# Neptune-Crypto/twenty-first

Hardware: AMD Instinct MI355X
Metric: goldilocks_ntt_gfelts_per_s (higher is better)
Workload: dtype u64

## Files before the change

### include/tf_hip.h

```cpp
#ifndef TF_HIP_H
#define TF_HIP_H

#include <stddef.h>
#include <stdint.h>

#ifdef __cplusplus
extern "C" {
#endif

enum tf_status {
    TF_OK = 0,
    TF_ERR_TOO_FEW_LEAFS = 1,
    TF_ERR_INCORRECT_NUMBER_OF_LEAFS = 2,
    TF_ERR_TREE_TOO_HIGH = 3,
    TF_ERR_LEN_NOT_POWER_OF_TWO = 4,
    TF_ERR_LEN_TOO_LARGE = 5,
    TF_ERR_ORDER_NOT_ABOVE_DEGREE = 6,
    TF_ERR_NULL_POINTER = 7,
    TF_ERR_NO_DEVICE = 8,
    TF_ERR_HIP = 9,
    TF_ERR_OUT_OF_MEMORY = 10,
    TF_ERR_LEAF_INDEX_INVALID = 11,
    TF_ERR_INVERSE_OF_ZERO = 12,
    TF_ERR_BUFFER_TOO_SMALL = 13,
// ... 333 lines not shown
    TF_FIELD_OP_ADD_SUB2 = 4,
    TF_FIELD_OP_ADD_SUB_LAZY2 = 5,
    TF_FIELD_OP_ADD_LAZY4 = 6,
    TF_FIELD_OP_SUB_LAZY4 = 7,
    TF_FIELD_OP_MONT_MUL2 = 8,
    TF_FIELD_OP_MONT_MUL3 = 9,
    TF_FIELD_OP_MONT_MUL4 = 10,
    TF_FIELD_OP_CANONICAL = 11,
    TF_FIELD_OP_MX_FOLD4_CANON = 12,
    TF_FIELD_OP_MX_FOLD4_LAZY = 13,
    TF_FIELD_OP_MX_FOLD2 = 14,
    TF_FIELD_OP_COUNT = 15
};
int tf_debug_field_op_dev(int op, const uint64_t *d_a, const uint64_t *d_b, uint64_t *d_out0, uint64_t *d_out1, size_t count, void *stream);

enum { TF_NTT_NETWORK_FORM_COUNT = 42 };
int tf_debug_ntt_network_dev(int form, uint64_t *d_x, size_t count, void *stream);
void tf_debug_ntt_network_config(int *lazy, int *asm_bfly, int *asm_pow2, int *pow2_wide);

#ifdef __cplusplus
}
#endif
#endif
```

### twenty-first_amd/csrc/ntt_kernels.h

```cpp
#pragma once

#include <type_traits>

#include "gl64.h"
#include "ntt_args.h"
#include "ntt_network.h"

namespace tfk {

using gl::u32;
using gl::u64;

struct NttPassArgs {
    const u64* in;
    u64* out;
    const u64* inner_tw;
    const u64* post_tw;
    const u64* pre_scale;
    long long n_out;
    const u64* in2;
    const u64* post_scale;
    long long js_i0, js_i1, js_i2, js_c, js_k;
    long long n_coeffs;
    long long ps_i1;
    long long ib0, ib1, ib2, ob0, ob1, ob2;
    long long in_cs_hi, out_cs_hi;
    long long in_rs, out_rs;
    long long tw_rs;
    long long ps_rs;
    u32 d1, d2;
    u32 d01;
// ... 47 lines not shown
    return ((u64)v[1] << 32) | v[0];
}
__device__ __forceinline__ u64 buf_load_tab(__amdgpu_buffer_rsrc_t r, u32 voff, u32 soff) {
    const tf_v2u v = __builtin_amdgcn_raw_buffer_load_b64(r, voff, soff, 0);
    return ((u64)v[1] << 32) | v[0];
}
template <int AUX = TF_STORE_AUX>
__device__ __forceinline__ void buf_store(__amdgpu_buffer_rsrc_t r, u32 voff, u32 soff, u64 x) {
    tf_v2u v;
    v[0] = (u32)x;
    v[1] = (u32)(x >> 32);
    __builtin_amdgcn_raw_buffer_store_b64(v, r, voff, soff, AUX);
}


template <bool INV, int Q0, bool TRUNC = false, bool SCALED = false>
__device__ __forceinline__ void tail_p5(u64 (&x)[32], bool act, char* obase, u32 toff, long long out_rs_bytes, int qlim = 32,
                                        const char* sbase = nullptr, u32 soff = 0, long long s_rs_bytes = 0, bool nt = false) {
    DitRange<INV, 5, Q0, Q0 + 4, false>::run(x);
    if (act) {
        const __amdgpu_buffer_rsrc_t ro = buf_rsrc(obase);
        if constexpr (SCALED) {
            u64 w[8];
#pragma unroll
            for (int i = 0; i < 4; ++i) {
                w[i] = *reinterpret_cast<const u64*>(sbase + (long long)(32 * (Q0 + i)) * s_rs_bytes + soff);
                w[4 + i] = *reinterpret_cast<const u64*>(sbase + (long long)(32 * (Q0 + i + 16)) * s_rs_bytes + soff);
            }
#pragma unroll
            for (int i = 0; i < 4; ++i) gl::mont_mul2(x[Q0 + i], w[i], x[Q0 + i + 16], w[4 + i], x[Q0 + i], x[Q0 + i + 16]);
        }
        (void)nt;
#pragma unroll
// ... 195 lines not shown
        }
    }
    const bool act_in = LAST1024 ? (c_in < ncv) : act;
    int ch_in = ch, cl_in = cl;
    if constexpr (LAST1024) {
        const int w = col0 + c_in + (col0 + c_in < 0 ? A.col_wrap : 0);
        const int e = (int)div_by_L((u32)w, L);
        ch_in = e - ch0, cl_in = w - e * L;
    }

    unsigned long long stamp[6];
    if constexpr (MODE == 3) stamp[0] = __builtin_readcyclecounter();
    u64 x[32];
#pragma unroll
    for (int q = 0; q < 32; ++q) x[q] = 0;
    constexpr bool LDS_TW = TF_LDS_TW && MODE == 0;
    u64* const ltw = lds + (LAST1024 ? kL1024ExchangeWords : 32 * s1_);
    if constexpr (LDS_TW) {
        if ((LAST1024 || R1024) || A.inner_tw) {
            const u64* itw = A.inner_tw + ((PRE2 || PRE4) ? (int)half * 1024 : 0);
            for (int i = t; i < 32 * P2; i += blockDim.x) ltw[(i >> 5) * kLdsTwStride + (i & 31)] = itw[i];
            __syncthreads();
        }
    }
    __builtin_amdgcn_s_setprio(TF_PRIO_LOAD);
    if constexpr (MODE == 1) {
#pragma unroll
        for (int q = 0; q < 32; ++q) x[q] = (u64)(t * 32 + q) * 0x9e3779b97f4a7c15ULL >> 1;
#ifdef TF_AB_BUILD
    } else if (PRE4 && act_in) {
// ... 131 lines not shown
        } else {
#pragma unroll
        for (int q = 0; q < 32; ++q) x[q] = ld(slot_off(q));
#pragma unroll
        for (int q0 = 0; q0 < 32; q0 += 8) {
            u64 w[8];
#pragma unroll
            for (int i = 0; i < 8; ++i) w[i] = ld(slot_off(q0 + i) + poff);
            scale8(w);
            if (q0 == 0) pre2_combine8<INV, 0>(x, w, half != 0);
            else if (q0 == 8) pre2_combine8<INV, 8>(x, w, half != 0);
            else if (q0 == 16) pre2_combine8<INV, 16>(x, w, half != 0);
            else pre2_combine8<INV, 24>(x, w, half != 0);
        }
        }
    } else if (act_in) {
        const u32 toff = (u32)(((long long)ch_in * A.in_cs_hi + cl_in + (long long)g_in * A.in_rs) * 8);
        const char* base = reinterpret_cast<const char*>(in);
        if constexpr ((LAST1024 || COLP) && SCALE != 1) {
            const __amdgpu_buffer_rsrc_t ri = buf_rsrc(in);
#pragma unroll
            for (int q = 0; q < 32; ++q) x[q] = buf_load<LAST1024 ? TF_AUX_LAST_LOAD : TF_LOAD_AUX>(ri, toff, (u32)((long long)(brev5(q) << p2) * A.in_rs * 8));
        } else
#pragma unroll
        for (int q = 0; q < 32; ++q) {
            const long long ur = (long long)(brev5(q) << p2);
            const u64* ptr = reinterpret_cast<const u64*>(base + ur * A.in_rs * 8 + toff);
            if constexpr (SCALE == 1) {
                const long long j = (ur + g) * A.ps_rs + (A.ps_col ? bcol : 0);
                if (A.n_coeffs < 0 || j < A.n_coeffs) x[q] = *ptr;
// ... 44 lines not shown
    __builtin_amdgcn_s_setprio(0);
    if constexpr (MODE != 2 && !(PRE2 && TF_PRE2_BURST16 == 2 && SCALE != 1)) {
        dit_half<INV, 0, LAZY1>(x);
        __builtin_amdgcn_sched_barrier(0);
    }
    if constexpr (MODE == 3) {
        stamp[1] = __builtin_readcyclecounter();
        asm volatile("s_waitcnt vmcnt(0)" ::: "memory");
        stamp[2] = __builtin_readcyclecounter();
    }
    if constexpr (MODE != 2) {
        dit_half<INV, 16, LAZY1>(x);
        dit_level<INV, 5, LAZY1>(x);
        if ((LAST1024 || R1024) || A.inner_tw) {
            const u64* tw = LDS_TW ? ltw + g_in * kLdsTwStride : A.inner_tw + g_in * 32;
#pragma unroll
            for (int q = 0; q < 32; q += 4) mul4_inplace(x, q, tw[q], tw[q + 1], tw[q + 2], tw[q + 3]);
        }
    }
    if constexpr (MODE == 3) { asm volatile("" :: "v"(x[0]), "v"(x[31])); stamp[3] = __builtin_readcyclecounter(); }
    if constexpr (LAST1024) {
        constexpr int S1 = kL1024S1, CS = kL1024CS;
        const int wround = c_in >> 3, wcc = c_in & 7, rround = c >> 3, rcc = c & 7;
        u64* wr = lds + wcc * CS + g_in;
        const u64* rd = lds + g * S1 + rcc * CS;
        const int nr = (A.nc + 7) >> 3;
#pragma unroll 1
        for (int r = 0; r < nr; ++r) {
            if (r) __syncthreads();
            if (wround == r) {
#pragma unroll
                for (int q = 0; q < 32; ++q) wr[q * S1] = x[q];
// ... 20 lines not shown
            if (myround == r) {
#pragma unroll
                for (int q = 0; q < 32; ++q) {
                    const int s = q >> p2;
                    const int gbr = q & (P2 - 1);
                    const int gg = p2 ? (int)(__brev((unsigned)gbr) >> (32 - p2)) : 0;
                    const int k1 = g + (s << p2);
                    x[q] = rd[k1 * s1_ + gg * s2_];
                }
            }
        }
    }
    if constexpr (MODE == 3) { asm volatile("" :: "v"(x[0]), "v"(x[31])); stamp[4] = __builtin_readcyclecounter(); }
    __builtin_amdgcn_s_setprio(TF_PRIO_STEP2);
    if constexpr (LAST1024) {
        dit_half<INV, 0>(x);
        dit_half<INV, 16>(x);
        const u32 toff = (u32)(((long long)ch * A.out_cs_hi + cl + (long long)g * A.out_rs) * 8);
        char* base = reinterpret_cast<char*>(out);
        if constexpr (SCALE == 2) {
            long long j0 = (long long)i0 * A.js_i0 + (long long)i1 * A.js_i1 + (long long)(ch0 + ch) * A.js_c + (long long)g * A.js_k;
            if constexpr (PRE2) j0 += (long long)half * A.pre2_js_off;
            const char* sb = reinterpret_cast<const char*>(A.post_scale);
            const u32 soff = (u32)(j0 * 8);
            tail_p5<INV, 0, false, true>(x, act, base, toff, A.out_rs * 8, 32, sb, soff, A.js_k * 8);
            tail_p5<INV, 4, false, true>(x, act, base, toff, A.out_rs * 8, 32, sb, soff, A.js_k * 8);
            tail_p5<INV, 8, false, true>(x, act, base, toff, A.out_rs * 8, 32, sb, soff, A.js_k * 8);
            tail_p5<INV, 12, false, true>(x, act, base, toff, A.out_rs * 8, 32, sb, soff, A.js_k * 8);
            return;
        }
        if (A.n_out >= 0) {
            const long long j0 = (long long)i0 * A.js_i0 + (long long)i1 * A.js_i1 + (long long)(ch0 + ch) * A.js_c + (long long)g * A.js_k;
            const long long rem = A.n_out - j0, step = 32 * A.js_k;
            const int qlim = rem <= 0 ? 0 : (int)min(32ll, (rem + step - 1) / step);
            tail_p5<INV, 0, true>(x, act, base, toff, A.out_rs * 8, qlim);
            tail_p5<INV, 4, true>(x, act, base, toff, A.out_rs * 8, qlim);
            tail_p5<INV, 8, true>(x, act, base, toff, A.out_rs * 8, qlim);
            tail_p5<INV, 12, true>(x, act, base, toff, A.out_rs * 8, qlim);
            return;
        }
        const bool nts = (A.nt & 2) != 0;
        tail_p5<INV, 0>(x, act, base, toff, A.out_rs * 8, 32, nullptr, 0, 0, nts);
        tail_p5<INV, 4>(x, act, base, toff, A.out_rs * 8, 32, nullptr, 0, 0, nts);
        tail_p5<INV, 8>(x, act, base, toff, A.out_rs * 8, 32, nullptr, 0, 0, nts);
        tail_p5<INV, 12>(x, act, base, toff, A.out_rs * 8, 32, nullptr, 0, 0, nts);
        return;
    }
    if constexpr (MODE != 2) {
        if (p2 >= 1) dit_level<INV, 1, LAZY2>(x);
        if (p2 >= 2) dit_level<INV, 2, LAZY2>(x);
        if (p2 >= 3) dit_level<INV, 3, LAZY2>(x);
        if (p2 >= 4) dit_level<INV, 4, LAZY2>(x);
        if (p2 >= 5) dit_level<INV, 5, LAZY2>(x);
    }
    if constexpr (MODE == 1) {
        u64 acc = 0;
#pragma unroll
        for (int q = 0; q < 32; ++q) acc ^= x[q];
        if (acc == 0x123456789abcdefULL) out[t] = acc;
    } else if (act) {
// ... 939 lines not shown
```

### twenty-first_amd/csrc/ntt_network.h

```cpp
#pragma once

#include "gl64.h"

namespace tfk {

using gl::u32;
using gl::u64;

template <bool INV, int LVL, int J>
struct TwExp {
    static constexpr int fwd = ((39 << (6 - LVL)) * J) % 192;
    static constexpr int value = INV ? (192 - fwd) % 192 : fwd;
};

#ifndef TF_ASM_BFLY
#define TF_ASM_BFLY 1
#endif
#ifndef TF_LDS_TW
#define TF_LDS_TW 1
#endif
constexpr int kLdsTwStride = 34;
constexpr int kR1024Nc = 16, kR1024Cpr = 8, kR1024Rounds = 2, kR1024S1 = 264;
constexpr int kL1024S1 = 273, kL1024CS = 34;
constexpr int kL1024ExchangeWords = ((31 * kL1024S1 + 7 * kL1024CS + 32 + 1) / 2) * 2;
#ifndef TF_LAZY
#define TF_LAZY 1
#endif

template <bool INV, int LVL, int I>
struct Bf {
    static constexpr int H = 1 << (LVL - 1);
    static constexpr int j = I % H;
    static constexpr int ia = (I / H) * 2 * H + j;
    static constexpr int ib = ia + H;
    static constexpr int E = TwExp<INV, LVL, j>::value;
    static constexpr bool neg = gl::Pow2Mul<E>::negate;
};

template <int E, bool LAZY_IN>
__device__ __forceinline__ u64 tw_operand(u64 b) {
    if constexpr (E % 192 == 0) {
// ... 143 lines not shown
        if constexpr (I + 2 < END) DitRange<INV, LVL, I + 2, END, LAZY>::run(x);
#endif
    }
};
template <bool INV, int LVL, bool LAZY = false, int WIDE = TF_POW2_WIDE>
__device__ __forceinline__ void dit_level(u64 (&x)[32]) { DitRange<INV, LVL, 0, 16, LAZY && TF_LAZY, WIDE>::run(x); }

template <bool INV, int FIRST, bool LAZY = false, int WIDE = TF_POW2_WIDE>
__device__ __forceinline__ void dit_half(u64 (&x)[32]) {
    DitRange<INV, 1, FIRST / 2, FIRST / 2 + 8, LAZY && TF_LAZY, WIDE>::run(x);
    DitRange<INV, 2, FIRST / 2, FIRST / 2 + 8, LAZY && TF_LAZY, WIDE>::run(x);
    DitRange<INV, 3, FIRST / 2, FIRST / 2 + 8, LAZY && TF_LAZY, WIDE>::run(x);
    DitRange<INV, 4, FIRST / 2, FIRST / 2 + 8, LAZY && TF_LAZY, WIDE>::run(x);
}

__device__ __forceinline__ void mul4_inplace(u64 (&x)[32], int q0, u64 w0, u64 w1, u64 w2, u64 w3) {
    const u64 a4[4] = {x[q0], x[q0 + 1], x[q0 + 2], x[q0 + 3]}, b4[4] = {w0, w1, w2, w3};
    u64 r4[4];
    gl::mont_mul4(a4, b4, r4);
    x[q0] = r4[0], x[q0 + 1] = r4[1], x[q0 + 2] = r4[2], x[q0 + 3] = r4[3];
}

}
```

### twenty-first_amd/csrc/tf_abi.hip

```cpp
#include "tf_temp.h"
#include "aux_kernels.h"

#include <functional>
#include <utility>

namespace tfi {

int h2d(u64* d, const u64* h, size_t words, hipStream_t s) {
    if (!words) return TF_OK;
    HIPCHK(hipMemcpyAsync(d, h, words * sizeof(u64), hipMemcpyHostToDevice, s));
    HIPCHK(hipStreamSynchronize(s));
    return TF_OK;
}

struct HostStreams {
    hipStream_t s[kMaxDevices] = {};
    ~HostStreams() {
        for (int d = 0; d < kMaxDevices; ++d)
            if (s[d]) (void)hipStreamDestroy(s[d]);
    }
};
hipStream_t host_stream() {
    thread_local HostStreams streams;
    int dev = 0;
// ... 212 lines not shown
} TF_ABI_CATCH

int tf_debug_field_op_dev(int op, const uint64_t* d_a, const uint64_t* d_b, uint64_t* d_out0, uint64_t* d_out1, size_t count, void* stream) try {
    if (op < 0 || op >= TF_FIELD_OP_COUNT || count > (size_t(1) << 32)) return TF_ERR_INVALID_ARGUMENT;
    if (count == 0) return TF_OK;
    if (!d_a || !d_out0 || (!d_b && op != TF_FIELD_OP_CANONICAL) || (!d_out1 && field_op_two_outputs(op))) return TF_ERR_NULL_POINTER;
    DeviceCtx* ctx = nullptr;
    int rc = current_ctx(&ctx);
    if (rc) return rc;
    debug_field_op_dev(op, d_a, d_b, d_out0, d_out1, count, static_cast<hipStream_t>(stream));
    HIPCHK(hipGetLastError());
    return TF_OK;
} TF_ABI_CATCH

int tf_debug_ntt_network_dev(int form, uint64_t* d_x, size_t count, void* stream) try {
    if (form < 0 || form >= TF_NTT_NETWORK_FORM_COUNT || count > (size_t(1) << 32)) return TF_ERR_INVALID_ARGUMENT;
    if (count % (size_t)debug_ntt_network_words(form)) return TF_ERR_INVALID_ARGUMENT;
    if (count == 0) return TF_OK;
    if (!d_x) return TF_ERR_NULL_POINTER;
    DeviceCtx* ctx = nullptr;
    int rc = current_ctx(&ctx);
    if (rc) return rc;
    debug_ntt_network_dev(form, reinterpret_cast<u64*>(d_x), count, static_cast<hipStream_t>(stream));
    HIPCHK(hipGetLastError());
    return TF_OK;
} TF_ABI_CATCH

void tf_debug_ntt_network_config(int* lazy, int* asm_bfly, int* asm_pow2, int* pow2_wide) { debug_ntt_network_config(lazy, asm_bfly, asm_pow2, pow2_wide); }

#ifdef TF_AB_BUILD
int tf_debug_stamps(unsigned long long* host_out, size_t words) try {
// ... 947 lines not shown
```

### twenty-first_amd/csrc/tf_ntt.hip

```cpp
#include "tf_temp.h"
#include "ntt_kernels.h"

namespace tfi {


thread_local std::string t_last_error;

int hip_fail(hipError_t e, const char* what, const char* file, int line) {
    char buf[512];
    snprintf(buf, sizeof(buf), "%s failed: %s (%s:%d)", what, hipGetErrorString(e), file, line);
    t_last_error = buf;
    (void)hipGetLastError();
    if (e == hipErrorNoDevice || e == hipErrorInvalidDevice || e == hipErrorInsufficientDriver || e == hipErrorNotInitialized)
        return TF_ERR_NO_DEVICE;
    if (e == hipErrorOutOfMemory || e == hipErrorMemoryAllocation) return TF_ERR_OUT_OF_MEMORY;
    return TF_ERR_HIP;
}

int abi_caught(const char* what, int status) noexcept {
    try {
        t_last_error = std::string("C++ exception at the C ABI: ") + (what ? what : "?");
    } catch (...) {
    }
    return status;
// ... 215 lines not shown
    u64 acc = gl::ONE;
    for (size_t i = 0; i < nlo; ++i) {
        (*lo)[i] = acc;
        acc = gl::mont_mul(acc, base);
    }
    u64 step = acc;
    acc = gl::ONE;
    for (size_t i = 0; i < nhi; ++i) {
        (*hi)[i] = acc;
        acc = gl::mont_mul(acc, step);
    }
    *h_out = h;
}


int get_inner_table(DeviceCtx* ctx, int a, bool inverse, int scale_log_n, const u64** out, int pre = 1, const u64** stw_out = nullptr) {
    const int p2 = a - 5;
    if (stw_out) *stw_out = nullptr;
    if (p2 == 0 && scale_log_n == 0) {
        *out = nullptr;
        return TF_OK;
    }
    const u64 key = make_key(TAG_INNER, a, inverse, scale_log_n, pre > 1 ? pre - 1 : 0);
    std::lock_guard<std::mutex> lk(ctx->mu);
    const int P2 = 1 << p2;
    auto it = ctx->tables.find(key);
    if (it != ctx->tables.end()) {
        *out = it->second;
        if (stw_out && pre == 4) *stw_out = it->second + size_t(P2) * 32 * 4;
        return TF_OK;
    }
    u64 w = root_of_unity_mont(a);
    if (inverse) w = gl::mont_inverse(w);
    u64 scale = gl::ONE;
    if (scale_log_n) scale = gl::mont_inverse(gl::to_mont(u64(1) << scale_log_n));
    std::vector<u64> t(size_t(P2) * 32);
    u64 wg = gl::ONE;
    for (int g = 0; g < P2; ++g) {
        u64 acc = scale;
        for (int k = 0; k < 32; ++k) {
            t[size_t(g) * 32 + k] = acc;
            acc = gl::mont_mul(acc, wg);
        }
        wg = gl::mont_mul(wg, w);
// ... 11 lines not shown
            }
            wq = gl::mont_mul(wq, wp);
        }
        if (pre == 4) {
            const u64 w128 = gl::mont_pow(wp, u64(P2));
            for (int h = 0; h < 2; ++h) {
                const u64 step = gl::mont_pow(w128, u64(2 * h + 1));
                u64 acc = gl::ONE;
                for (int i = 0; i < 32; ++i) {
                    t[size_t(P2) * 32 * 4 + size_t(h) * 32 + i] = acc;
                    acc = gl::mont_mul(acc, step);
                }
            }
        }
    }
    u64* d = nullptr;
    int rc = upload_table(t, &d);
    if (rc) return rc;
    ctx->tables[key] = d;
    *out = d;
    if (stw_out && pre == 4) *stw_out = d + size_t(P2) * 32 * 4;
    return TF_OK;
}

constexpr int kMaxCachedPostLog = 28;
constexpr int kAlwaysCachedPostLog = 22;
int get_post_table(DeviceCtx* ctx, int log_m, int a, bool inverse, hipStream_t stream, const u64** out, DevTemp* own) {
    bool temp = log_m > kMaxCachedPostLog;
    const u64 key = make_key(TAG_POST, log_m, a, inverse, 0);
    std::unique_lock<std::mutex> lk(ctx->mu);
    if (!temp) {
        auto it = ctx->tables.find(key);
        if (it != ctx->tables.end()) {
            *out = it->second;
            return TF_OK;
        }
// ... 829 lines not shown
    A.n_coeffs = c.n_coeffs;
    A.in_bs = c.in_bs;
    A.out_bs = c.out_bs;
    A.count = (long long)c.batch * c.L;
    A.scale = (c.inverse && c.log_n > 0) ? gl::mont_inverse(gl::to_mont(u64(c.n))) : 0;
    A.log_n = c.log_n;
    A.L = c.L;
    const long long blocks = (A.count + 255) / 256;
    hipLaunchKernelGGL(tfk::ntt_tiny_kernel, dim3((unsigned)blocks), dim3(256), 0, c.stream, A);
    HIPCHK(hipGetLastError());
    return TF_OK;
}

int run_row(const NttCall& c, const NttPlan& plan) {
    const u64* inner = nullptr;
    TRY(get_inner_table(c.ctx, c.log_n, c.inverse, c.inverse ? c.log_n : 0, &inner));
    const size_t max_batch = size_t(1) << 24;
    for (size_t b0 = 0; b0 < c.batch; b0 += max_batch) {
        const size_t nb = std::min(max_batch, c.batch - b0);
        Launch l = plan_row_pass(plan, c.in + b0 * c.in_bs, c.out + b0 * c.out_bs, c.in_bs, c.out_bs, nb, c.log_n, c.L);
        l.a.inner_tw = inner;
        l.a.pre_scale = c.pre_scale;
        l.a.post_scale = c.post_scale;
        l.a.n_coeffs = c.n_coeffs;
        l.a.in2 = c.in2 ? c.in2 + b0 * c.in_bs : nullptr;
        TRY(launch_pass(l, c.inverse, c.stream));
    }
    return TF_OK;
}

class TileScope {
public:
    TileScope(DeviceCtx* ctx, hipStream_t stream) : ctx_(ctx), stream_(stream) {}
    TileScope(const TileScope&) = delete;
    TileScope& operator=(const TileScope&) = delete;
    ~TileScope() { (void)finish(); }
// ... 50 lines not shown
    bool forked_ = false;
    hipEvent_t ev_fork_ = nullptr, ev_join_[kMaxPipe] = {nullptr, nullptr, nullptr, nullptr};
};

int run_passes(const NttCall& c, const NttPlan& plan) {
    DeviceCtx* const ctx = c.ctx;
    const int P = plan.P, L = c.L, log_n = c.log_n;
    const int (&a)[4] = plan.a;
    const bool (&pre2)[4] = plan.pre2;
    const bool inverse = c.inverse, c8 = plan.c8, pre4_last = plan.pre4_last;
    const size_t n = c.n, cosets = c.cosets;
    const long long n_coeffs = c.n_coeffs, n_out = c.n_out;
    const u64 *const pre_scale = c.pre_scale, *const post_scale = c.post_scale;
    const u64* pre4_stw = nullptr;
    const u64* inner[4] = {nullptr, nullptr, nullptr, nullptr};
    for (int i = 0; i < P; ++i) {
        const bool p4 = pre4_last && i == P - 1;
        TRY(get_inner_table(ctx, (pre2[i] || p4) ? 10 : a[i], inverse, (i == P - 1 && inverse) ? log_n : 0, &inner[i], p4 ? 4 : (pre2[i] ? 2 : 1),
                            p4 ? &pre4_stw : nullptr));
    }
    const u64* post[3] = {nullptr, nullptr, nullptr};
    const u64* post_u = nullptr;
    DevTemp post_own[3] = {DevTemp(c.stream), DevTemp(c.stream), DevTemp(c.stream)}, post_u_own(c.stream);
    {
        int rest = log_n;
        for (int i = 0; i + 1 < P; ++i) {
            if (i == 0 && c8 && pre_scale) {
                TRY(get_scaled_post_table(ctx, rest, a[i], *c.coset_offset, c.stream, &post[i], &post_own[i]));
                TRY(get_post_table(ctx, rest, a[i], inverse, c.stream, &post_u, &post_u_own));
            } else {
                TRY(get_post_table(ctx, rest, a[i], inverse, c.stream, &post[i], &post_own[i]));
            }
            rest -= a[i];
        }
// ... 26 lines not shown
        const size_t nb = std::min(tb, c.batch - b0);
        hipStream_t const stream = K > 1 ? side[tile_no % K] : c.stream;
        u64* const scratch = K > 1 ? tiles.scratch() + (tile_no % K) * tb * (size_t)sbs : tiles.scratch();
        const u64* tin = c.in + (long long)b0 * c.in_bs;
        u64* tout = c.out + (long long)b0 * c.out_bs;
        const u64* src = tin;
        long long src_bs = c.in_bs;
        long long outer = 1, B = (long long)n;
        for (int i = 0; i + 1 < P && rc == TF_OK; ++i) {
            B >>= a[i];
            const bool to_scratch = i == P - 2;
            u64* dst = to_scratch ? scratch : (n_out >= 0 ? const_cast<u64*>(tin) : tout);
            const long long dst_bs = to_scratch ? sbs : (n_out >= 0 ? c.in_bs : c.out_bs);
            Launch p = plan_column_pass(plan, src, dst, src_bs, dst_bs, nb, (i == 0) ? (long long)cosets : outer, a[i], B, L, pre2[i]);
            p.a.inner_tw = inner[i];
            p.a.post_tw = post[i];
            p.a.post_tw_u = (i == 0 && post_u) ? post_u : nullptr;
            if (pre2[i]) {
                p.a.pre2_cp = pre_scale ? pre_scale + ((long long)(n / 2) < n_coeffs ? (long long)(n / 2) : 0) : nullptr;
            }
            if (i == 0 && src != dst) p.a.nt = g_nt.load(std::memory_order_relaxed) & 1;
            if (i == 0) {
                p.a.pre_scale = pre_scale;
                if (c8 && pre_scale) p.a.ps_col = 0;
                p.a.n_coeffs = n_coeffs;
                p.a.in2 = c.in2 ? c.in2 + (long long)b0 * c.in_bs : nullptr;
                if (cosets > 1) {
                    p.a.ib1 = 0;
                    p.a.ob1 = B * L;
                    p.a.out_rs = (long long)cosets * B * L;
                    p.a.ps_i1 = n_coeffs;
                }
                outer = (long long)cosets;
            }
            rc = launch_pass(p, inverse, stream);
            src = dst;
            src_bs = dst_bs;
            outer <<= a[i];
        }
        if (rc) break;
        if (P < 4) {
            Launch pl = plan_transpose_pass(plan, scratch, tout, sbs, c.out_bs, nb, a[P - 1], N[0] * (long long)cosets, P == 3 ? N[1] : 1, L, 0,
                                            plan.words, pre4_last ? 4 : (pre2[P - 1] ? 2 : 1));
            pl.a.inner_tw = inner[P - 1];
            pl.a.pre4_stw = pre4_last ? pre4_stw : nullptr;
            pl.a.post_scale = post_scale;
            pl.a.n_out = n_out;
            pl.a.nt = g_nt.load(std::memory_order_relaxed) & 2;
            if (plan.plain1024 && !pre4_last && pl.a.nc == 16 && !no_col_shift && (unsigned long long)n * L * sizeof(u64) < (1ull << 32)) {
                pl.a.col_shift0 = (int)((reinterpret_cast<uintptr_t>(tout) / sizeof(u64)) & 15);
                pl.a.col_shift_i0 = (int)(c.out_bs & 15);
                pl.a.col_wrap = pl.a.col_limit;
            }
            rc = launch_pass(pl, inverse, stream);
        } else {
            for (size_t b = 0; b < nb && rc == TF_OK; ++b) {
                Launch pl = plan_transpose_pass(plan, scratch + (long long)b * sbs, tout + (long long)b * c.out_bs, sbs, c.out_bs, 1, a[3], N[0],
                                                N[1] * N[2], L, N[1]);
                pl.a.inner_tw = inner[3];
                pl.a.post_scale = post_scale;
                rc = launch_pass(pl, inverse, stream);
            }
        }
    }
    const int jrc = tiles.finish();
    return jrc ? jrc : rc;
}

int run_ntt(DeviceCtx* ctx, const u64* in, u64* out, long long in_bs, long long out_bs, size_t n, size_t batch, int L,
            bool inverse, const u64* pre_scale, long long n_coeffs, hipStream_t stream, const u64* post_scale,
            size_t cosets, const u64* in2, long long n_out, const u64* coset_offset) {
    if (n == 0 || batch == 0) return TF_OK;
    NttShape s;
    s.n = n, s.batch = batch, s.L = L, s.inverse = inverse, s.cosets = cosets, s.n_coeffs = n_coeffs, s.n_out = n_out;
// ... 49 lines not shown
        rc = run_ntt(ctx, d_coeffs, d_out, (long long)n_coeffs * L, (long long)order * L, order / cosets, batch, L, false, pw,
                     (long long)n_coeffs, s, nullptr, cosets);
    } else {
        rc = get_pow_table(ctx, offset_raw, n_coeffs, s, &pw, &temp);
        if (rc) return rc;
        rc = run_ntt(ctx, d_coeffs, d_out, (long long)n_coeffs * L, (long long)order * L, order, batch, L, false, pw,
                     (long long)n_coeffs, s, nullptr, 1, nullptr, -1, &offset_raw);
    }
    release_pow_table(ctx, pw, temp, s);
    return rc;
}


constexpr int kNetLevels = 6, kNetTail5 = 26, kNetLat = 28, kNetPre2 = 34, kNetC8 = 38;
static_assert(kNetC8 + 4 == TF_NTT_NETWORK_FORM_COUNT, "include/tf_hip.h lists the forms");
constexpr int net_form_words(int form) { return form >= kNetPre2 ? 64 : 32; }

template <bool INV, bool LAZY, int WIDE>
__device__ __forceinline__ void net32_form(u64 (&x)[32]) {
    tfk::dit_half<INV, 0, LAZY, WIDE>(x);
    tfk::dit_half<INV, 16, LAZY, WIDE>(x);
    tfk::dit_level<INV, 5, LAZY, WIDE>(x);
}
template <bool INV, bool LAZY, int P2, int LVL = 1>
__device__ __forceinline__ void levels_form(u64 (&x)[32]) {
    if constexpr (LVL <= P2) {
        tfk::dit_level<INV, LVL, LAZY>(x);
        levels_form<INV, LAZY, P2, LVL + 1>(x);
    }
}

template <int FORM>
__global__ void __launch_bounds__(256) ntt_network_form_kernel(u64* d, unsigned long long blocks, int half) {
    constexpr int B = net_form_words(FORM);
    const unsigned long long t = (unsigned long long)blockIdx.x * blockDim.x + threadIdx.x;
    if (t >= blocks) return;
    u64* const p = d + t * B;
    u64 x[32];
#pragma unroll
    for (int q = 0; q < 32; ++q) x[q] = p[q];
    if constexpr (FORM < kNetLevels) {
        constexpr bool INV = (FORM & 1) != 0;
        constexpr int V = FORM >> 1;
        if constexpr (V == 0) net32_form<INV, true, TF_POW2_WIDE>(x);
        else if constexpr (V == 1) net32_form<INV, true, 2>(x);
        else net32_form<INV, false, TF_POW2_WIDE>(x);
    } else if constexpr (FORM < kNetTail5) {
        constexpr int K = FORM - kNetLevels;
        levels_form<(K & 1) != 0, ((K >> 1) & 1) != 0, (K >> 2) + 1>(x);
    } else if constexpr (FORM < kNetLat) {
        constexpr bool INV = ((FORM - kNetTail5) & 1) != 0;
        tfk::dit_half<INV, 0>(x);
        tfk::dit_half<INV, 16>(x);
        tfk::DitRange<INV, 5, 0, 4, false>::run(x);
        tfk::DitRange<INV, 5, 4, 8, false>::run(x);
        tfk::DitRange<INV, 5, 8, 12, false>::run(x);
// ... 29 lines not shown
            tfk::c8_combine8<INV, 8>(x, wb, half != 0);
#pragma unroll
            for (int i = 0; i < 8; ++i) wa[i] = p[48 + i], wb[i] = p[56 + i];
            tfk::c8_combine8<INV, 16>(x, wa, half != 0);
            tfk::c8_combine8<INV, 24>(x, wb, half != 0);
            if (half) tfk::pre2_shift<INV>(x);
            levels_form<INV, true, 5>(x);
        }
    }
#pragma unroll
    for (int q = 0; q < 32; ++q) p[q] = x[q];
}

template <int FORM>
void network_form_launch(u64* d_x, size_t blocks, hipStream_t s) {
    const int half = FORM >= kNetPre2 ? ((FORM - kNetPre2) >> 1) & 1 : 0;
    hipLaunchKernelGGL(ntt_network_form_kernel<FORM>, dim3((unsigned)((blocks + 255) / 256)), dim3(256), 0, s, d_x, (unsigned long long)blocks, half);
}
template <int... FORM>
void network_form_dispatch(int form, u64* d_x, size_t blocks, hipStream_t s, std::integer_sequence<int, FORM...>) {
    using Fn = void (*)(u64*, size_t, hipStream_t);
    static const Fn table[] = {&network_form_launch<FORM>...};
    table[form](d_x, blocks, s);
}
int debug_ntt_network_words(int form) { return net_form_words(form); }
void debug_ntt_network_dev(int form, u64* d_x, size_t count, hipStream_t s) {
    network_form_dispatch(form, d_x, count / (size_t)net_form_words(form), s, std::make_integer_sequence<int, TF_NTT_NETWORK_FORM_COUNT>{});
}
void debug_ntt_network_config(int* lazy, int* asm_bfly, int* asm_pow2, int* pow2_wide) {
    if (lazy) *lazy = TF_LAZY;
    if (asm_bfly) *asm_bfly = TF_ASM_BFLY;
    if (asm_pow2) *asm_pow2 = TF_ASM_POW2;
    if (pow2_wide) *pow2_wide = TF_POW2_WIDE;
}


}
```

### twenty-first_amd/device.py

```python
from __future__ import annotations

import ctypes as C

from . import _lib


def _chk(rc, where):
    from . import _check

    _check(rc, where)


def _t(t, name="tensor"):
    import torch

    if not isinstance(t, torch.Tensor) or not t.is_cuda or not t.is_contiguous() or t.dtype not in (torch.int64, torch.uint64):
        raise TypeError(f"{name} must be a contiguous CUDA int64/uint64 tensor of raw Montgomery words")
    return t


def _stream(stream):
    import torch

    s = stream if stream is not None else torch.cuda.current_stream()
# ... 45 lines not shown

NETWORK_FORMS = {}
for _inv in (0, 1):
    _d = "inv" if _inv else "fwd"
    for _v, _name in enumerate(("lazy", "lazy_wide2", "canonical")):
        NETWORK_FORMS[f"NET32_{_d}_{_name}"] = (0 + 2 * _v + _inv, 32)
    for _p2 in range(1, 6):
        for _lazy in (0, 1):
            NETWORK_FORMS[f"LEVELS{_p2}_{_d}_{'lazy' if _lazy else 'canonical'}"] = (6 + 4 * (_p2 - 1) + 2 * _lazy + _inv, 32)
    NETWORK_FORMS[f"TAIL5_{_d}"] = (26 + _inv, 32)
    for _logr in (1, 2, 3):
        NETWORK_FORMS[f"LAT{_logr}_{_d}"] = (28 + 2 * (_logr - 1) + _inv, 32)
    for _half in (0, 1):
        NETWORK_FORMS[f"PRE2_{_d}_half{_half}"] = (34 + 2 * _half + _inv, 64)
        NETWORK_FORMS[f"C8_{_d}_half{_half}"] = (38 + 2 * _half + _inv, 64)


def debug_ntt_network_(form: str, x, stream=None) -> None:
    code, words = NETWORK_FORMS[form]
    x = _t(x, "x")
    _need(x.numel() % words == 0, f"{form} works on whole blocks of {words} words")
    _chk(_lib.lib().tf_debug_ntt_network_dev(code, _p(x), x.numel(), _stream(stream)), "debug_ntt_network")


def debug_ntt_network_config() -> dict:
    v = [C.c_int(-1) for _ in range(4)]
    _lib.lib().tf_debug_ntt_network_config(*[C.byref(i) for i in v])
    return dict(zip(("lazy", "asm_bfly", "asm_pow2", "pow2_wide"), (i.value for i in v)))


def ntt_(x, n: int, batch: int = 1, width: int = 1, inverse: bool = False, stream=None) -> None:
    x = _t(x, "x")
    _width(width)
    if x.numel() != n * batch * width:
# ... 798 lines not shown
```

Before: 146.8.

## Use lazy reduction in final NTT tail, skip unit inner twiddle, add full-load path

Runs the last-1024 tail's dit_half levels in lazy (non-canonical) form and canonicalizes only the words entering level 5. When every group's first inner twiddle is one, the host records that flag and the kernel skips that multiply, replacing it with a canonicalization. It also adds an unconditional full 32-word buffer-load path with a scheduling barrier when at least 16 columns are active. The aim is to cut modular reductions and multiplies, at the cost of extra host bookkeeping (mutex and map) and new debug network forms for testing.

```diff
diff --git a/include/tf_hip.h b/include/tf_hip.h
--- a/include/tf_hip.h
+++ b/include/tf_hip.h
@@ -371,7 +371,7 @@
 };
 int tf_debug_field_op_dev(int op, const uint64_t *d_a, const uint64_t *d_b, uint64_t *d_out0, uint64_t *d_out1, size_t count, void *stream);
 
-enum { TF_NTT_NETWORK_FORM_COUNT = 42 };
+enum { TF_NTT_NETWORK_FORM_COUNT = 42, TF_NTT_NETWORK_FORM2_BASE = 64, TF_NTT_NETWORK_FORM2_COUNT = 4 };
 int tf_debug_ntt_network_dev(int form, uint64_t *d_x, size_t count, void *stream);
 void tf_debug_ntt_network_config(int *lazy, int *asm_bfly, int *asm_pow2, int *pow2_wide);
 
diff --git a/twenty-first_amd/csrc/ntt_kernels.h b/twenty-first_amd/csrc/ntt_kernels.h
--- a/twenty-first_amd/csrc/ntt_kernels.h
+++ b/twenty-first_amd/csrc/ntt_kernels.h
@@ -15,6 +15,7 @@
     const u64* in;
     u64* out;
     const u64* inner_tw;
+    int inner_one0;
     const u64* post_tw;
     const u64* pre_scale;
     long long n_out;
@@ -92,9 +93,10 @@
 }
 
 
-template <bool INV, int Q0, bool TRUNC = false, bool SCALED = false>
+template <bool INV, int Q0, bool TRUNC = false, bool SCALED = false, bool LAZY_IN = false>
 __device__ __forceinline__ void tail_p5(u64 (&x)[32], bool act, char* obase, u32 toff, long long out_rs_bytes, int qlim = 32,
                                         const char* sbase = nullptr, u32 soff = 0, long long s_rs_bytes = 0, bool nt = false) {
+    if constexpr (LAZY_IN) level5_entry<Q0>(x);
     DitRange<INV, 5, Q0, Q0 + 4, false>::run(x);
     if (act) {
         const __amdgpu_buffer_rsrc_t ro = buf_rsrc(obase);
@@ -320,6 +322,7 @@
     u64 x[32];
 #pragma unroll
     for (int q = 0; q < 32; ++q) x[q] = 0;
+    constexpr bool FULLP = (LAST1024 || R1024) && !PRE2 && !PRE4 && SCALE != 1 && MODE != 1;
     constexpr bool LDS_TW = TF_LDS_TW && MODE == 0;
     u64* const ltw = lds + (LAST1024 ? kL1024ExchangeWords : 32 * s1_);
     if constexpr (LDS_TW) {
@@ -481,6 +484,12 @@
             else pre2_combine8<INV, 24>(x, w, half != 0);
         }
         }
+    } else if (FULLP && ncv >= 16) {
+        const u32 toff = (u32)(((long long)ch_in * A.in_cs_hi + cl_in + (long long)g_in * A.in_rs) * 8);
+        const __amdgpu_buffer_rsrc_t ri = buf_rsrc(in);
+#pragma unroll
+        for (int q = 0; q < 32; ++q) x[q] = buf_load<LAST1024 ? TF_AUX_LAST_LOAD : TF_LOAD_AUX>(ri, toff, (u32)((long long)(brev5(q) << p2) * A.in_rs * 8));
+        __builtin_amdgcn_sched_barrier(0);
     } else if (act_in) {
         const u32 toff = (u32)(((long long)ch_in * A.in_cs_hi + cl_in + (long long)g_in * A.in_rs) * 8);
         const char* base = reinterpret_cast<const char*>(in);
@@ -555,8 +564,7 @@
         dit_level<INV, 5, LAZY1>(x);
         if ((LAST1024 || R1024) || A.inner_tw) {
             const u64* tw = LDS_TW ? ltw + g_in * kLdsTwStride : A.inner_tw + g_in * 32;
-#pragma unroll
-            for (int q = 0; q < 32; q += 4) mul4_inplace(x, q, tw[q], tw[q + 1], tw[q + 2], tw[q + 3]);
+            inner_twiddle32(x, tw, A.inner_one0 && half == 0);
         }
     }
     if constexpr (MODE == 3) { asm volatile("" :: "v"(x[0]), "v"(x[31])); stamp[3] = __builtin_readcyclecounter(); }
@@ -607,8 +615,9 @@
     if constexpr (MODE == 3) { asm volatile("" :: "v"(x[0]), "v"(x[31])); stamp[4] = __builtin_readcyclecounter(); }
     __builtin_amdgcn_s_setprio(TF_PRIO_STEP2);
     if constexpr (LAST1024) {
-        dit_half<INV, 0>(x);
-        dit_half<INV, 16>(x);
+        constexpr bool LT = TF_LAZY_TAIL && TF_LAZY;
+        dit_half<INV, 0, LT>(x);
+        dit_half<INV, 16, LT>(x);
         const u32 toff = (u32)(((long long)ch * A.out_cs_hi + cl + (long long)g * A.out_rs) * 8);
         char* base = reinterpret_cast<char*>(out);
         if constexpr (SCALE == 2) {
@@ -616,27 +625,27 @@
             if constexpr (PRE2) j0 += (long long)half * A.pre2_js_off;
             const char* sb = reinterpret_cast<const char*>(A.post_scale);
             const u32 soff = (u32)(j0 * 8);
-            tail_p5<INV, 0, false, true>(x, act, base, toff, A.out_rs * 8, 32, sb, soff, A.js_k * 8);
-            tail_p5<INV, 4, false, true>(x, act, base, toff, A.out_rs * 8, 32, sb, soff, A.js_k * 8);
-            tail_p5<INV, 8, false, true>(x, act, base, toff, A.out_rs * 8, 32, sb, soff, A.js_k * 8);
-            tail_p5<INV, 12, false, true>(x, act, base, toff, A.out_rs * 8, 32, sb, soff, A.js_k * 8);
+            tail_p5<INV, 0, false, true, LT>(x, act, base, toff, A.out_rs * 8, 32, sb, soff, A.js_k * 8);
+            tail_p5<INV, 4, false, true, LT>(x, act, base, toff, A.out_rs * 8, 32, sb, soff, A.js_k * 8);
+            tail_p5<INV, 8, false, true, LT>(x, act, base, toff, A.out_rs * 8, 32, sb, soff, A.js_k * 8);
+            tail_p5<INV, 12, false, true, LT>(x, act, base, toff, A.out_rs * 8, 32, sb, soff, A.js_k * 8);
             return;
         }
         if (A.n_out >= 0) {
             const long long j0 = (long long)i0 * A.js_i0 + (long long)i1 * A.js_i1 + (long long)(ch0 + ch) * A.js_c + (long long)g * A.js_k;
             const long long rem = A.n_out - j0, step = 32 * A.js_k;
             const int qlim = rem <= 0 ? 0 : (int)min(32ll, (rem + step - 1) / step);
-            tail_p5<INV, 0, true>(x, act, base, toff, A.out_rs * 8, qlim);
-            tail_p5<INV, 4, true>(x, act, base, toff, A.out_rs * 8, qlim);
-            tail_p5<INV, 8, true>(x, act, base, toff, A.out_rs * 8, qlim);
-            tail_p5<INV, 12, true>(x, act, base, toff, A.out_rs * 8, qlim);
+            tail_p5<INV, 0, true, false, LT>(x, act, base, toff, A.out_rs * 8, qlim);
+            tail_p5<INV, 4, true, false, LT>(x, act, base, toff, A.out_rs * 8, qlim);
+            tail_p5<INV, 8, true, false, LT>(x, act, base, toff, A.out_rs * 8, qlim);
+            tail_p5<INV, 12, true, false, LT>(x, act, base, toff, A.out_rs * 8, qlim);
             return;
         }
         const bool nts = (A.nt & 2) != 0;
-        tail_p5<INV, 0>(x, act, base, toff, A.out_rs * 8, 32, nullptr, 0, 0, nts);
-        tail_p5<INV, 4>(x, act, base, toff, A.out_rs * 8, 32, nullptr, 0, 0, nts);
-        tail_p5<INV, 8>(x, act, base, toff, A.out_rs * 8, 32, nullptr, 0, 0, nts);
-        tail_p5<INV, 12>(x, act, base, toff, A.out_rs * 8, 32, nullptr, 0, 0, nts);
+        tail_p5<INV, 0, false, false, LT>(x, act, base, toff, A.out_rs * 8, 32, nullptr, 0, 0, nts);
+        tail_p5<INV, 4, false, false, LT>(x, act, base, toff, A.out_rs * 8, 32, nullptr, 0, 0, nts);
+        tail_p5<INV, 8, false, false, LT>(x, act, base, toff, A.out_rs * 8, 32, nullptr, 0, 0, nts);
+        tail_p5<INV, 12, false, false, LT>(x, act, base, toff, A.out_rs * 8, 32, nullptr, 0, 0, nts);
         return;
     }
     if constexpr (MODE != 2) {
diff --git a/twenty-first_amd/csrc/ntt_network.h b/twenty-first_amd/csrc/ntt_network.h
--- a/twenty-first_amd/csrc/ntt_network.h
+++ b/twenty-first_amd/csrc/ntt_network.h
@@ -25,6 +25,9 @@
 constexpr int kL1024ExchangeWords = ((31 * kL1024S1 + 7 * kL1024CS + 32 + 1) / 2) * 2;
 #ifndef TF_LAZY
 #define TF_LAZY 1
+#endif
+#ifndef TF_LAZY_TAIL
+#define TF_LAZY_TAIL 1
 #endif
 
 template <bool INV, int LVL, int I>
@@ -198,6 +201,21 @@
     DitRange<INV, 4, FIRST / 2, FIRST / 2 + 8, LAZY && TF_LAZY, WIDE>::run(x);
 }
 
+__device__ __forceinline__ u64 canonical_word(u64 b) {
+#if TF_ASM_POW2
+    return gl::canonical_asm(b);
+#else
+    return gl::add(b, 0);
+#endif
+}
+
+template <int Q0>
+__device__ __forceinline__ void level5_entry(u64 (&x)[32]) {
+#pragma unroll
+    for (int i = 0; i < 4; ++i) x[Q0 + i] = canonical_word(x[Q0 + i]);
+    if constexpr (Q0 == 0) x[16] = canonical_word(x[16]);
+}
+
 __device__ __forceinline__ void mul4_inplace(u64 (&x)[32], int q0, u64 w0, u64 w1, u64 w2, u64 w3) {
     const u64 a4[4] = {x[q0], x[q0 + 1], x[q0 + 2], x[q0 + 3]}, b4[4] = {w0, w1, w2, w3};
     u64 r4[4];
@@ -205,4 +223,21 @@
     x[q0] = r4[0], x[q0 + 1] = r4[1], x[q0 + 2] = r4[2], x[q0 + 3] = r4[3];
 }
 
-}
+#ifndef TF_INNER_ONE0
+#define TF_INNER_ONE0 1
+#endif
+__device__ __forceinline__ void inner_twiddle32(u64 (&x)[32], const u64* tw, bool one0) {
+    if (TF_INNER_ONE0 && one0) {
+        x[0] = canonical_word(x[0]);
+        const u64 a3[3] = {x[1], x[2], x[3]}, b3[3] = {tw[1], tw[2], tw[3]};
+        u64 r3[3];
+        gl::mont_mul3(a3, b3, r3);
+        x[1] = r3[0], x[2] = r3[1], x[3] = r3[2];
+    } else {
+        mul4_inplace(x, 0, tw[0], tw[1], tw[2], tw[3]);
+    }
+#pragma unroll
+    for (int q = 4; q < 32; q += 4) mul4_inplace(x, q, tw[q], tw[q + 1], tw[q + 2], tw[q + 3]);
+}
+
+}
diff --git a/twenty-first_amd/csrc/tf_abi.hip b/twenty-first_amd/csrc/tf_abi.hip
--- a/twenty-first_amd/csrc/tf_abi.hip
+++ b/twenty-first_amd/csrc/tf_abi.hip
@@ -250,7 +250,8 @@
 } TF_ABI_CATCH
 
 int tf_debug_ntt_network_dev(int form, uint64_t* d_x, size_t count, void* stream) try {
-    if (form < 0 || form >= TF_NTT_NETWORK_FORM_COUNT || count > (size_t(1) << 32)) return TF_ERR_INVALID_ARGUMENT;
+    const bool form2 = form >= TF_NTT_NETWORK_FORM2_BASE && form < TF_NTT_NETWORK_FORM2_BASE + TF_NTT_NETWORK_FORM2_COUNT;
+    if (form < 0 || (form >= TF_NTT_NETWORK_FORM_COUNT && !form2) || count > (size_t(1) << 32)) return TF_ERR_INVALID_ARGUMENT;
     if (count % (size_t)debug_ntt_network_words(form)) return TF_ERR_INVALID_ARGUMENT;
     if (count == 0) return TF_OK;
     if (!d_x) return TF_ERR_NULL_POINTER;
diff --git a/twenty-first_amd/csrc/tf_ntt.hip b/twenty-first_amd/csrc/tf_ntt.hip
--- a/twenty-first_amd/csrc/tf_ntt.hip
+++ b/twenty-first_amd/csrc/tf_ntt.hip
@@ -253,9 +253,13 @@
 }
 
 
-int get_inner_table(DeviceCtx* ctx, int a, bool inverse, int scale_log_n, const u64** out, int pre = 1, const u64** stw_out = nullptr) {
+int get_inner_table(DeviceCtx* ctx, int a, bool inverse, int scale_log_n, const u64** out, int pre = 1, const u64** stw_out = nullptr,
+                    int* one0_out = nullptr) {
+    static std::mutex one0_mu;
+    static std::map<u64, int> one0_of_key;
     const int p2 = a - 5;
     if (stw_out) *stw_out = nullptr;
+    if (one0_out) *one0_out = 0;
     if (p2 == 0 && scale_log_n == 0) {
         *out = nullptr;
         return TF_OK;
@@ -267,6 +271,11 @@
     if (it != ctx->tables.end()) {
         *out = it->second;
         if (stw_out && pre == 4) *stw_out = it->second + size_t(P2) * 32 * 4;
+        if (one0_out) {
+            std::lock_guard<std::mutex> lk1(one0_mu);
+            const auto f = one0_of_key.find(key);
+            *one0_out = f != one0_of_key.end() ? f->second : 0;
+        }
         return TF_OK;
     }
     u64 w = root_of_unity_mont(a);
@@ -308,12 +317,19 @@
             }
         }
     }
+    int one0 = 1;
+    for (int g = 0; g < P2; ++g) one0 &= t[size_t(g) * 32] == gl::ONE;
     u64* d = nullptr;
     int rc = upload_table(t, &d);
     if (rc) return rc;
     ctx->tables[key] = d;
+    {
+        std::lock_guard<std::mutex> lk1(one0_mu);
+        one0_of_key[key] = one0;
+    }
     *out = d;
     if (stw_out && pre == 4) *stw_out = d + size_t(P2) * 32 * 4;
+    if (one0_out) *one0_out = one0;
     return TF_OK;
 }
 
@@ -1173,12 +1189,14 @@
 
 int run_row(const NttCall& c, const NttPlan& plan) {
     const u64* inner = nullptr;
-    TRY(get_inner_table(c.ctx, c.log_n, c.inverse, c.inverse ? c.log_n : 0, &inner));
+    int inner_one0 = 0;
+    TRY(get_inner_table(c.ctx, c.log_n, c.inverse, c.inverse ? c.log_n : 0, &inner, 1, nullptr, &inner_one0));
     const size_t max_batch = size_t(1) << 24;
     for (size_t b0 = 0; b0 < c.batch; b0 += max_batch) {
         const size_t nb = std::min(max_batch, c.batch - b0);
         Launch l = plan_row_pass(plan, c.in + b0 * c.in_bs, c.out + b0 * c.out_bs, c.in_bs, c.out_bs, nb, c.log_n, c.L);
         l.a.inner_tw = inner;
+        l.a.inner_one0 = inner_one0;
         l.a.pre_scale = c.pre_scale;
         l.a.post_scale = c.post_scale;
         l.a.n_coeffs = c.n_coeffs;
@@ -1259,10 +1277,11 @@
     const u64 *const pre_scale = c.pre_scale, *const post_scale = c.post_scale;
     const u64* pre4_stw = nullptr;
     const u64* inner[4] = {nullptr, nullptr, nullptr, nullptr};
+    int inner_one0[4] = {0, 0, 0, 0};
     for (int i = 0; i < P; ++i) {
         const bool p4 = pre4_last && i == P - 1;
         TRY(get_inner_table(ctx, (pre2[i] || p4) ? 10 : a[i], inverse, (i == P - 1 && inverse) ? log_n : 0, &inner[i], p4 ? 4 : (pre2[i] ? 2 : 1),
-                            p4 ? &pre4_stw : nullptr));
+                            p4 ? &pre4_stw : nullptr, &inner_one0[i]));
     }
     const u64* post[3] = {nullptr, nullptr, nullptr};
     const u64* post_u = nullptr;
@@ -1319,6 +1338,7 @@
             const long long dst_bs = to_scratch ? sbs : (n_out >= 0 ? c.in_bs : c.out_bs);
             Launch p = plan_column_pass(plan, src, dst, src_bs, dst_bs, nb, (i == 0) ? (long long)cosets : outer, a[i], B, L, pre2[i]);
             p.a.inner_tw = inner[i];
+            p.a.inner_one0 = inner_one0[i];
             p.a.post_tw = post[i];
             p.a.post_tw_u = (i == 0 && post_u) ? post_u : nullptr;
             if (pre2[i]) {
@@ -1348,6 +1368,7 @@
             Launch pl = plan_transpose_pass(plan, scratch, tout, sbs, c.out_bs, nb, a[P - 1], N[0] * (long long)cosets, P == 3 ? N[1] : 1, L, 0,
                                             plan.words, pre4_last ? 4 : (pre2[P - 1] ? 2 : 1));
             pl.a.inner_tw = inner[P - 1];
+            pl.a.inner_one0 = inner_one0[P - 1];
             pl.a.pre4_stw = pre4_last ? pre4_stw : nullptr;
             pl.a.post_scale = post_scale;
             pl.a.n_out = n_out;
@@ -1363,6 +1384,7 @@
                 Launch pl = plan_transpose_pass(plan, scratch + (long long)b * sbs, tout + (long long)b * c.out_bs, sbs, c.out_bs, 1, a[3], N[0],
                                                 N[1] * N[2], L, N[1]);
                 pl.a.inner_tw = inner[3];
+                pl.a.inner_one0 = inner_one0[3];
                 pl.a.post_scale = post_scale;
                 rc = launch_pass(pl, inverse, stream);
             }
@@ -1442,7 +1464,9 @@
 
 constexpr int kNetLevels = 6, kNetTail5 = 26, kNetLat = 28, kNetPre2 = 34, kNetC8 = 38;
 static_assert(kNetC8 + 4 == TF_NTT_NETWORK_FORM_COUNT, "include/tf_hip.h lists the forms");
-constexpr int net_form_words(int form) { return form >= kNetPre2 ? 64 : 32; }
+constexpr int kNet2LTail5 = TF_NTT_NETWORK_FORM2_BASE, kNet2One0 = kNet2LTail5 + 2;
+static_assert(kNet2One0 + 2 == TF_NTT_NETWORK_FORM2_BASE + TF_NTT_NETWORK_FORM2_COUNT && TF_NTT_NETWORK_FORM2_BASE > TF_NTT_NETWORK_FORM_COUNT, "include/tf_hip.h lists the forms");
+constexpr int net_form_words(int form) { return (form >= kNetPre2 && form < TF_NTT_NETWORK_FORM_COUNT) || form >= kNet2One0 ? 64 : 32; }
 
 template <bool INV, bool LAZY, int WIDE>
 __device__ __forceinline__ void net32_form(u64 (&x)[32]) {
@@ -1467,7 +1491,27 @@
     u64 x[32];
 #pragma unroll
     for (int q = 0; q < 32; ++q) x[q] = p[q];
-    if constexpr (FORM < kNetLevels) {
+    if constexpr (FORM >= kNet2One0) {
+        constexpr bool INV = ((FORM - kNet2One0) & 1) != 0;
+        net32_form<INV, true, TF_POW2_WIDE>(x);
+        u64 w[32];
+#pragma unroll
+        for (int q = 0; q < 32; ++q) w[q] = p[32 + q];
+        tfk::inner_twiddle32(x, w, half == 0);
+    } else if constexpr (FORM >= kNet2LTail5) {
+        constexpr bool INV = ((FORM - kNet2LTail5) & 1) != 0;
+        constexpr bool LT = TF_LAZY_TAIL && TF_LAZY;
+        tfk::dit_half<INV, 0, LT>(x);
+        tfk::dit_half<INV, 16, LT>(x);
+        if constexpr (LT) tfk::level5_entry<0>(x);
+        tfk::DitRange<INV, 5, 0, 4, false>::run(x);
+        if constexpr (LT) tfk::level5_entry<4>(x);
+        tfk::DitRange<INV, 5, 4, 8, false>::run(x);
+        if constexpr (LT) tfk::level5_entry<8>(x);
+        tfk::DitRange<INV, 5, 8, 12, false>::run(x);
+        if constexpr (LT) tfk::level5_entry<12>(x);
+        tfk::DitRange<INV, 5, 12, 16, false>::run(x);
+    } else if constexpr (FORM < kNetLevels) {
         constexpr bool INV = (FORM & 1) != 0;
         constexpr int V = FORM >> 1;
         if constexpr (V == 0) net32_form<INV, true, TF_POW2_WIDE>(x);
@@ -1527,14 +1571,17 @@
 
 template <int FORM>
 void network_form_launch(u64* d_x, size_t blocks, hipStream_t s) {
-    const int half = FORM >= kNetPre2 ? ((FORM - kNetPre2) >> 1) & 1 : 0;
+    const int half = (FORM >= kNetPre2 && FORM < TF_NTT_NETWORK_FORM_COUNT) ? ((FORM - kNetPre2) >> 1) & 1 : 0;
     hipLaunchKernelGGL(ntt_network_form_kernel<FORM>, dim3((unsigned)((blocks + 255) / 256)), dim3(256), 0, s, d_x, (unsigned long long)blocks, half);
 }
 template <int... FORM>
 void network_form_dispatch(int form, u64* d_x, size_t blocks, hipStream_t s, std::integer_sequence<int, FORM...>) {
     using Fn = void (*)(u64*, size_t, hipStream_t);
     static const Fn table[] = {&network_form_launch<FORM>...};
-    table[form](d_x, blocks, s);
+    static const Fn table2[] = {&network_form_launch<kNet2LTail5>, &network_form_launch<kNet2LTail5 + 1>, &network_form_launch<kNet2One0>,
+                                &network_form_launch<kNet2One0 + 1>};
+    if (form >= TF_NTT_NETWORK_FORM2_BASE) table2[form - TF_NTT_NETWORK_FORM2_BASE](d_x, blocks, s);
+    else table[form](d_x, blocks, s);
 }
 int debug_ntt_network_words(int form) { return net_form_words(form); }
 void debug_ntt_network_dev(int form, u64* d_x, size_t count, hipStream_t s) {
diff --git a/twenty-first_amd/device.py b/twenty-first_amd/device.py
--- a/twenty-first_amd/device.py
+++ b/twenty-first_amd/device.py
@@ -83,10 +83,11 @@
     for _half in (0, 1):
         NETWORK_FORMS[f"PRE2_{_d}_half{_half}"] = (34 + 2 * _half + _inv, 64)
         NETWORK_FORMS[f"C8_{_d}_half{_half}"] = (38 + 2 * _half + _inv, 64)
+NETWORK_FORMS2 = {"LTAIL5_fwd": (64, 32), "LTAIL5_inv": (65, 32), "ONE0_fwd": (66, 64), "ONE0_inv": (67, 64)}
 
 
 def debug_ntt_network_(form: str, x, stream=None) -> None:
-    code, words = NETWORK_FORMS[form]
+    code, words = NETWORK_FORMS[form] if form in NETWORK_FORMS else NETWORK_FORMS2[form]
     x = _t(x, "x")
     _need(x.numel() % words == 0, f"{form} works on whole blocks of {words} words")
     _chk(_lib.lib().tf_debug_ntt_network_dev(code, _p(x), x.numel(), _stream(stream)), "debug_ntt_network")
```

Measured after the change: 147.7, median of 6. About the same (+0.6%).
